# marksgraham/ddpm-ood

Measured on AMD Instinct MI355X. Metric: reconstructions/sec (whole node), FashionMNIST 32x32, higher is better.
Workload: dtype f32 (split-f16 MFMA products, fp32 accumulate)

## Files before the change

### ddpm_ood_amd/csrc/api.hip

```cpp
#include <stdarg.h>
#include <string.h>

#include <map>
#include <string>
#include <vector>

#include "common.h"

namespace ddpm {

static thread_local char g_err[512] = "";

void set_error(const char *fmt, ...) {
  va_list ap;
  va_start(ap, fmt);
  vsnprintf(g_err, sizeof(g_err), fmt, ap);
  va_end(ap);
}

static Switches g_sw;
static bool g_sw_loaded = false;
static unsigned g_sw_epoch = 0;
unsigned switch_epoch() { return g_sw_epoch; }
static int env_int(const char *name, int dflt) {
  const char *v = getenv(name);
  return v && *v ? atoi(v) : dflt;
}
static long env_long(const char *name, long dflt) {
  const char *v = getenv(name);
  return v && *v ? atol(v) : dflt;
}
static bool env_set(const char *name) { return getenv(name) != nullptr; }
static void load_switches() {
  const bool keep = g_sw.split_f16;
  Switches n;
  n.conv_wino44 = env_int("DDPM_CONV_WINO44", 1);
  n.wino44_f16x3 = env_int("DDPM_WINO44_F16X3", 1) != 0;
  n.wino44_split = env_int("DDPM_WINO44_SPLIT", 4);
  n.wino_split = env_int("DDPM_WINO_SPLIT", 8);
  n.w44h_xitem = env_int("DDPM_W44H_XITEM", 1);
  n.w44r_serp = env_int("DDPM_W44R_SERP", 0);
  n.wino44_xmap = env_int("DDPM_WINO44_XMAP", -1);
  n.up_wino44h = env_int("DDPM_UP_WINO44H", 1) != 0;
  n.down_s2h = env_int("DDPM_DOWN_S2H", 1);
  n.conv1x1_f16x3 = env_int("DDPM_CONV1X1_F16X3", 1) != 0;
  n.attn_f16x3 = env_int("DDPM_ATTN_F16X3", 1) != 0;
  n.wgrad_f16x3 = env_int("DDPM_WGRAD_F16X3", 1) != 0;
  n.attn_fa = env_int("DDPM_ATTN_FA", 1);
  n.conv_d3s = env_int("DDPM_CONV_D3S", 1);
  n.d1s_maxpx = env_int("DDPM_D1S_MAXPX", 16384);
  n.conv_splitk = env_int("DDPM_CONV_SPLITK", 1) != 0;
  n.conv_winograd = env_int("DDPM_CONV_WINOGRAD", 1) != 0;
  n.linear_skinny = env_int("DDPM_LINEAR_SKINNY", 1) != 0;
  n.conv1x1_dma = env_int("DDPM_CONV1X1_DMA", 1) != 0;
  n.gn_fused = env_int("DDPM_GN_FUSED", 1) != 0;
  n.attn_waves8 = env_int("DDPM_ATTN_WAVES", 8) != 4;
  n.convin_fast = env_int("DDPM_CONVIN_FAST", 1) != 0;
  n.convout_wave = env_int("DDPM_CONVOUT_WAVE", 1) != 0;
  n.convout_w16_maxwg = env_long("DDPM_CONVOUT_W16_MAXWG", -1);
  n.convin_blocks_per_cu = env_long("DDPM_CONVIN_BLOCKS_PER_CU", 8);
  n.gn_fwd_reg = env_int("DDPM_GN_FWD_REG", 1) != 0;
  n.gn_bwd_reg = env_int("DDPM_GN_BWD_REG", 1) != 0;
  n.gemm_v4 = env_int("DDPM_GEMM_V4", 1) != 0;
  n.gemm_f16x3 = env_int("DDPM_GEMM_F16X3", 1) != 0;
  n.wgrad_staged = env_int("DDPM_WGRAD_STAGED", 1) != 0;
  n.wgrad_waves8 = env_int("DDPM_WGRAD_WAVES", 8) != 4;
  n.gn_wave = env_int("DDPM_GN_WAVE", 1) != 0;
  n.conv1x1_dma_min_wg = env_long("DDPM_CONV1X1_DMA_MIN_WG", -1);
  n.conv1x1_xcd = env_int("DDPM_CONV1X1_XCD", 1) != 0;
  n.conv1x1_presplit = env_int("DDPM_CONV1X1_PRESPLIT", 1) != 0;
  n.conv_min_wg128 = env_long("DDPM_CONV_MIN_WG128", 512);
  n.conv_debug = env_set("DDPM_CONV_DEBUG");
  n.prof_shapes = env_set("DDPM_PROF_SHAPES");
  n.split_f16 = g_sw_loaded ? keep : true;
  g_sw = n;
  g_sw_loaded = true;
  g_sw_epoch += 1;
}
const Switches &sw() {
  if (!g_sw_loaded) load_switches();
  return g_sw;
}

static unsigned *g_status[64] = {};
unsigned *status_word() {
  int dev = 0;
  if (hipGetDevice(&dev) != hipSuccess || dev < 0 || dev >= 64) return nullptr;
  if (!g_status[dev]) {
    unsigned *p = nullptr;
    if (hipMalloc(&p, 256) != hipSuccess) return nullptr;
    if (hipMemset(p, 0, 256) != hipSuccess) {
      (void)hipFree(p);
      return nullptr;
    }
    g_status[dev] = p;
  }
  return g_status[dev];
}

struct ProfRec {
  hipEvent_t a, b;
  std::string kernel;
  double flops, bytes;
};
bool g_prof_on = false;
static std::vector<ProfRec> g_recs;

void prof_begin(hipStream_t s, const char *kernel, double flops, double bytes) {
  ProfRec r{nullptr, nullptr, std::string(kernel), flops, bytes};
  if (hipEventCreate(&r.a) != hipSuccess || hipEventCreate(&r.b) != hipSuccess) return;
  (void)hipEventRecord(r.a, s);
  g_recs.push_back(r);
}

void prof_end(hipStream_t s) {
  if (!g_recs.empty()) (void)hipEventRecord(g_recs.back().b, s);
}

}

using namespace ddpm;

extern "C" int ddpm_prof_enable(int on) {
  g_prof_on = on != 0;
  return 0;
}

extern "C" int ddpm_prof_report(char *buf, size_t cap) {
  struct Agg { long n = 0; double ms = 0, flops = 0, bytes = 0; };
  std::map<std::string, Agg> agg;
  for (auto &r : g_recs) {
    float ms = 0.f;
    if (hipEventSynchronize(r.b) == hipSuccess && hipEventElapsedTime(&ms, r.a, r.b) == hipSuccess) {
      Agg &a = agg[r.kernel];
      a.n += 1; a.ms += ms; a.flops += r.flops; a.bytes += r.bytes;
    }
    (void)hipEventDestroy(r.a);
    (void)hipEventDestroy(r.b);
  }
  g_recs.clear();
  std::string out = "{";
  bool first = true;
  for (auto &kv : agg) {
    char line[768];
    snprintf(line, sizeof(line), "%s\"%s\": {\"launches\": %ld, \"ms\": %.6f, \"flops\": %.6e, \"bytes\": %.6e}",
             first ? "" : ", ", kv.first.c_str(), kv.second.n, kv.second.ms, kv.second.flops, kv.second.bytes);
    out += line;
    first = false;
  }
  out += "}";
  if (!buf || out.size() + 1 > cap) {
    set_error("prof_report: buffer too small (%zu needed)", out.size() + 1);
    return DDPM_EINVAL;
  }
  memcpy(buf, out.c_str(), out.size() + 1);
  return (int)out.size();
}

extern "C" int ddpm_reload_env(void) {
  load_switches();
  return 0;
}

extern "C" int ddpm_set_split_f16(int on) {
  (void)sw();
  const int was = g_sw.split_f16 ? 1 : 0;
  if ((on != 0) != g_sw.split_f16) g_sw_epoch += 1;
  g_sw.split_f16 = on != 0;
  return was;
}

extern "C" int ddpm_get_split_f16(void) { return sw().split_f16 ? 1 : 0; }

extern "C" int ddpm_split_f16_active(void) {
  const Switches &w = sw();
  const bool any = w.wino44_f16x3 || w.conv1x1_f16x3 || w.attn_f16x3 || w.down_s2h != 0 || w.conv_d3s != 0 || w.up_wino44h;
  return w.split_f16 && any ? 1 : 0;
}

extern "C" int ddpm_status_read(unsigned *word, int clear, ddpm_stream_t stream) {
  DDPM_CHECK_ARG(word != nullptr, "status_read: NULL pointer");
  unsigned *st = status_word();
  DDPM_CHECK_ARG(st != nullptr, "status_read: no status word on this device");
  hipError_t e = hipMemcpyAsync(word, st, sizeof(unsigned), hipMemcpyDeviceToHost, as_stream(stream));
  if (e == hipSuccess && clear) e = hipMemsetAsync(st, 0, sizeof(unsigned), as_stream(stream));
  if (e == hipSuccess) e = hipStreamSynchronize(as_stream(stream));
  if (e != hipSuccess) {
    set_error("status_read: %s", hipGetErrorString(e));
    return (int)e;
  }
  return 0;
}

extern "C" int ddpm_abi_version(void) { return DDPM_ABI_VERSION; }
extern "C" const char *ddpm_last_error(void) { return g_err; }

extern "C" int ddpm_conv_f32(const ddpm_conv_desc *d, ddpm_stream_t stream) {
  DDPM_CHECK_ARG(d != nullptr, "conv: descriptor is NULL");
  return conv_dispatch(*d, as_stream(stream));
}

extern "C" size_t ddpm_conv_scratch_floats(const ddpm_conv_desc *d) {
  if (!d) return 0;
  return conv_scratch_floats(*d);
}

extern "C" size_t ddpm_conv_s2h_weight_halves(int Cout, int Cin) { return conv_s2h_weight_halves(Cout, Cin); }

extern "C" int ddpm_pack_conv_s2h_weight(const float *w_raw, uint16_t *dst, int Cout, int Cin, ddpm_stream_t stream) {
  return launch_pack_conv_s2h_weight(w_raw, dst, Cout, Cin, as_stream(stream));
}

extern "C" size_t ddpm_conv_d3h_weight_halves(int Cout, int Cin) { return conv_d3h_weight_halves(Cout, Cin); }

extern "C" size_t ddpm_conv_d1s_weight_halves(int Cout, int Cin) { return conv_d1s_weight_halves(Cout, Cin); }

extern "C" int ddpm_pack_conv_d1s_weight(const float *w_raw, uint16_t *dst, int Cout, int Cin, int cout_offset, int Cout_total,
                                         ddpm_stream_t stream) {
  return launch_pack_conv_d1s_weight(w_raw, dst, Cout, Cin, cout_offset, Cout_total, as_stream(stream));
}

extern "C" int ddpm_pack_conv_d3h_weight(const float *w_raw, uint16_t *dst, int Cout, int Cin, ddpm_stream_t stream) {
  return launch_pack_conv_d3h_weight(w_raw, dst, Cout, Cin, as_stream(stream));
}

extern "C" size_t ddpm_conv1x1_h_weight_halves(int Cout, int Cin) { return conv1x1_h_weight_halves(Cout, Cin); }

extern "C" int ddpm_pack_conv1x1_h_weight(const float *w_raw, uint16_t *dst, int Cout, int Cin, ddpm_stream_t stream) {
  return launch_pack_conv1x1_h_weight(w_raw, dst, Cout, Cin, 0, Cout, as_stream(stream));
}

extern "C" int ddpm_conv_stats_parts(const ddpm_conv_desc *d) {
  if (!d) return 0;
  return conv_stats_parts(*d);
}

extern "C" size_t ddpm_packed_conv_weight_floats(int Cout, int Cin, int ksize) {
  return packed_conv_weight_floats(Cout, Cin, ksize);
}

extern "C" int ddpm_pack_conv_weight_f32(const float *w_raw, float *w_packed, int Cout, int Cin, int ksize,
                                         int cout_offset, int Cout_total, ddpm_stream_t stream) {
  DDPM_CHECK_ARG(w_raw && w_packed, "pack: NULL pointer");
  return launch_pack_conv_weight(w_raw, w_packed, Cout, Cin, ksize, cout_offset, Cout_total, as_stream(stream));
}

extern "C" int ddpm_pack_conv_weight_taps_f32(const float *w_raw, float *w_packed, int Cout, int Cin, int ksize,
                                              int src_taps, int tap_off, ddpm_stream_t stream) {
  DDPM_CHECK_ARG(w_raw && w_packed && src_taps >= ksize * ksize && tap_off >= 0 && tap_off + ksize * ksize <= src_taps,
                 "pack_taps: bad argument");
  return launch_pack_conv_weight(w_raw, w_packed, Cout, Cin, ksize, 0, Cout, as_stream(stream), src_taps, tap_off);
}

extern "C" int ddpm_pack_conv3d_weight_f32(const float *w_raw, float *w_packed, int Cout, int Cin, int ksize,
                                           ddpm_stream_t stream) {
  DDPM_CHECK_ARG(w_raw && w_packed && (ksize == 3 || ksize == 4), "pack_conv3d: NULL pointer or ksize not 3 / 4");
  const size_t slab = (size_t)Cout * Cin * ksize * ksize;
  for (int kd = 0; kd < ksize; ++kd) {
    const int rc = launch_pack_conv_weight(w_raw, w_packed + kd * slab, Cout, Cin, ksize, 0, Cout, as_stream(stream),
                                           ksize * ksize * ksize, ksize * ksize * kd);
    if (rc) return rc;
  }
  return 0;
}

extern "C" size_t ddpm_packed_convtr_weight_floats(int Cout, int Cin, int dims) {
  return packed_convT_weight_floats(Cout, Cin, dims);
}

extern "C" int ddpm_pack_convtr_weight_f32(const float *w_raw, float *w_packed, int Cin, int Cout, int dims,
                                          ddpm_stream_t stream) {
  DDPM_CHECK_ARG(w_raw && w_packed, "pack_convT: NULL pointer");
  return launch_pack_convT_weight(w_raw, w_packed, Cin, Cout, dims, as_stream(stream));
}

extern "C" int ddpm_conv3d_k4s2_cin1_f32(const float *in, const float *w, const float *bias, float *out, int B,
                                         int Cout, int D, int H, int W, int relu, ddpm_stream_t stream) {
  return launch_conv3d_k4s2_cin1(in, w, bias, out, B, Cout, D, H, W, relu, as_stream(stream));
}

extern "C" int ddpm_convtr3d_k4s2_cout1_f32(const float *in, const float *w, const float *bias, float *out, int B,
                                           int Cin, int D, int H, int W, ddpm_stream_t stream) {
  return launch_convT3d_k4s2_cout1(in, w, bias, out, B, Cin, D, H, W, as_stream(stream));
}

extern "C" size_t ddpm_wino_weight_floats(int Cout, int Cin) { return wino_weight_floats(Cout, Cin); }

extern "C" int ddpm_pack_wino_weight_f32(const float *w_raw, float *w_wino, int Cout, int Cin, ddpm_stream_t stream) {
  DDPM_CHECK_ARG(w_raw && w_wino, "wino pack: NULL pointer");
  return launch_pack_wino_weight(w_raw, w_wino, Cout, Cin, as_stream(stream));
}

extern "C" size_t ddpm_wino44_weight_floats(int Cout, int Cin) { return wino44_weight_floats(Cout, Cin); }

extern "C" int ddpm_pack_wino44_weight_f32(const float *w_raw, float *w_wino44, int Cout, int Cin, ddpm_stream_t stream) {
  DDPM_CHECK_ARG(w_raw && w_wino44, "wino44 pack: NULL pointer");
  return launch_pack_wino44_weight(w_raw, w_wino44, Cout, Cin, as_stream(stream));
}

extern "C" int ddpm_convnd_generic_f32(const float *in, const float *w, const float *bias, const float *residual, float *out,
                                       int B, int Cin, int Cout, int Di, int Hi, int Wi, int dims, int ksize, int stride,
                                       int pad, int transposed, int relu, ddpm_stream_t stream) {
  return launch_convnd_generic(in, w, bias, residual, out, B, Cin, Cout, Di, Hi, Wi, dims, ksize, stride, pad, transposed, relu,
                               as_stream(stream));
}

extern "C" size_t ddpm_wino44h_weight_halves(int Cout, int Cin) { return wino44h_weight_halves(Cout, Cin); }

extern "C" int ddpm_pack_wino44h_weight(const float *w_raw, uint16_t *w_wino44h, int Cout, int Cin, ddpm_stream_t stream) {
  DDPM_CHECK_ARG(w_raw && w_wino44h, "wino44h pack: NULL pointer");
  return launch_pack_wino44h_weight(w_raw, w_wino44h, Cout, Cin, as_stream(stream));
}

extern "C" int ddpm_pack_wino44h_weight3d(const float *w_raw, uint16_t *w_wino44h, int Cout, int Cin, ddpm_stream_t stream) {
  DDPM_CHECK_ARG(w_raw && w_wino44h, "wino44h 3d pack: NULL pointer");
  return launch_pack_wino44h_weight(w_raw, w_wino44h, Cout, Cin, as_stream(stream), 3);
}

extern "C" int ddpm_pack_wino44_weight3d_f32(const float *w_raw, float *w_wino44, int Cout, int Cin, ddpm_stream_t stream) {
  DDPM_CHECK_ARG(w_raw && w_wino44, "wino44 3d pack: NULL pointer");
  return launch_pack_wino44_weight(w_raw, w_wino44, Cout, Cin, as_stream(stream), 3);
}

extern "C" int ddpm_pack_wino3d_weight_f32(const float *w_raw, float *w_wino, int Cout, int Cin, ddpm_stream_t stream) {
  DDPM_CHECK_ARG(w_raw && w_wino, "wino3d pack: NULL pointer");
  return launch_pack_wino_weight(w_raw, w_wino, Cout, Cin, as_stream(stream), 3);
}

extern "C" size_t ddpm_folded_upsample_weight_floats(int Cout, int Cin) {
  return folded_upsample_weight_floats(Cout, Cin);
}

extern "C" int ddpm_fold_upsample_weight_f32(const float *w_raw, float *w_folded, int Cout, int Cin,
                                             ddpm_stream_t stream) {
  DDPM_CHECK_ARG(w_raw && w_folded, "fold: NULL pointer");
  return launch_fold_upsample_weight(w_raw, w_folded, Cout, Cin, as_stream(stream));
}

extern "C" int ddpm_gn_finalize_f32(const float *st1, int parts1, int C1, const float *st2, int parts2, int C2,
                                    const float *gamma, const float *beta, float *scale, float *shift, int B, int HW,
                                    int groups, float eps, ddpm_stream_t stream) {
  return launch_gn_finalize(st1, parts1, C1, st2, parts2, C2, gamma, beta, scale, shift, B, HW, groups, eps,
                            as_stream(stream));
}

extern "C" int ddpm_channel_stats_f32(const float *in, float *stats, int B, int C, int HW, ddpm_stream_t stream) {
  return launch_channel_stats(in, stats, B, C, HW, as_stream(stream));
}

extern "C" int ddpm_gn_scale_shift_f32(const float *in1, const float *in2, int C1, int C2, const float *gamma,
                                       const float *beta, float *scale, float *shift, int B, int HW, int groups,
                                       float eps, ddpm_stream_t stream) {
  return launch_gn_scale_shift(in1, in2, C1, C2, gamma, beta, scale, shift, B, HW, groups, eps, as_stream(stream));
}

extern "C" int ddpm_attention_f32(const float *qkv, const float *residual, float *out, int B, int C, int N,
                                  int num_heads, float scale, ddpm_stream_t stream) {
  return launch_attention(qkv, residual, out, B, C, N, num_heads, scale, as_stream(stream));
}

extern "C" size_t ddpm_attention_scratch_floats(int B, int C, int N, int num_heads) {
  return attention_fa_scratch_floats(B, C, N, num_heads);
}

extern "C" int ddpm_attention_ws_f32(const float *qkv, const float *residual, float *out, int B, int C, int N, int num_heads,
                                     float scale, float *scratch, size_t scratch_floats, ddpm_stream_t stream) {
  return launch_attention(qkv, residual, out, B, C, N, num_heads, scale, as_stream(stream), scratch, scratch_floats);
}

extern "C" int ddpm_attention_train_fwd_f32(const float *q, const float *k, const float *v, float *o, float *lse, int B, int C, int N,
                                            int num_heads, float scale, ddpm_stream_t stream) {
  return launch_attention_train_fwd(q, k, v, o, lse, B, C, N, num_heads, scale, as_stream(stream));
}

extern "C" int ddpm_attention_train_bwd_f32(const float *q, const float *k, const float *v, const float *o, const float *dout,
                                            const float *lse, float *delta, float *dq, float *dk, float *dv, int B, int C, int N,
                                            int num_heads, float scale, ddpm_stream_t stream) {
  return launch_attention_train_bwd(q, k, v, o, dout, lse, delta, dq, dk, dv, B, C, N, num_heads, scale, as_stream(stream));
}
```

### ddpm_ood_amd/csrc/common.h

```cpp
#pragma once
#include <hip/hip_runtime.h>
#include <stdint.h>
#include <stdio.h>
#include <string>

#include "../../include/ddpm_ood_hip.h"

namespace ddpm {

void set_error(const char *fmt, ...);

inline hipStream_t as_stream(ddpm_stream_t s) { return reinterpret_cast<hipStream_t>(s); }

#define DDPM_CHECK_ARG(cond, ...)                \
  do {                                           \
    if (!(cond)) {                               \
      ::ddpm::set_error(__VA_ARGS__);            \
      return DDPM_EINVAL;                        \
    }                                            \
  } while (0)

#define DDPM_CHECK_LAUNCH()                                                    \
  do {                                                                         \
    hipError_t e_ = hipGetLastError();                                         \
    if (e_ != hipSuccess) {                                                    \
      ::ddpm::set_error("%s:%d: %s", __FILE__, __LINE__, hipGetErrorString(e_)); \
      return (int)e_;                                                          \
    }                                                                          \
  } while (0)

constexpr int kWave = 64;

struct Switches {
  int conv_wino44 = 1;
  bool wino44_f16x3 = true;
  int wino44_split = 4;
  int wino_split = 8;
  int wino44_xmap = -1;
  int w44r_serp = 0;
  int w44h_xitem = 1;
  bool up_wino44h = true;
  int down_s2h = 1;
  bool conv1x1_f16x3 = true;
  bool attn_f16x3 = true;
  int d1s_maxpx = 16384;
  int conv_d3s = 1;
  int attn_fa = 1;
  bool conv_splitk = true;
  bool conv_winograd = true;
  bool linear_skinny = true;
  bool conv1x1_dma = true;
  bool gn_fused = true;
  bool attn_waves8 = true;
  bool convin_fast = true;
  bool convout_wave = true;
  long convout_w16_maxwg = -1;
  long convin_blocks_per_cu = 8;
  bool wgrad_f16x3 = true;
  bool gn_fwd_reg = true;
  bool gn_bwd_reg = true;
  bool gemm_v4 = true;
  bool gemm_f16x3 = true;
  bool wgrad_staged = true;
  bool wgrad_waves8 = true;
  bool gn_wave = true;
  long conv1x1_dma_min_wg = -1;
  bool conv1x1_xcd = true;
  bool conv1x1_presplit = true;
  long conv_min_wg128 = 512;
  bool conv_debug = false;
  bool prof_shapes = false;
  bool split_f16 = true;
};
const Switches &sw();
unsigned switch_epoch();
inline bool split_f16_on(bool family) { return family && sw().split_f16; }

unsigned *status_word();
__device__ __forceinline__ bool non_finite(float v) { return !(__builtin_fabsf(v) <= 3.402823466e+38f); }

__device__ __forceinline__ void philox_round(uint32_t (&c)[4], uint32_t (&k)[2]) {
  const uint64_t p0 = (uint64_t)0xD2511F53u * c[0], p1 = (uint64_t)0xCD9E8D57u * c[2];
  const uint32_t n0 = (uint32_t)(p1 >> 32) ^ c[1] ^ k[0], n1 = (uint32_t)p1, n2 = (uint32_t)(p0 >> 32) ^ c[3] ^ k[1], n3 = (uint32_t)p0;
  c[0] = n0; c[1] = n1; c[2] = n2; c[3] = n3;
  k[0] += 0x9E3779B9u;
  k[1] += 0xBB67AE85u;
}
__device__ __forceinline__ void philox_normal4(int64_t q, uint64_t stream, uint64_t seed, float (&z)[4]) {
  uint32_t c[4] = {(uint32_t)q, (uint32_t)((uint64_t)q >> 32), (uint32_t)stream, (uint32_t)(stream >> 32)};
  uint32_t k[2] = {(uint32_t)seed, (uint32_t)(seed >> 32)};
#pragma unroll
  for (int r = 0; r < 10; ++r) philox_round(c, k);
#pragma unroll
  for (int h = 0; h < 2; ++h) {
    const float u1 = ((float)c[2 * h] + 1.0f) * 2.3283064365386963e-10f;
    const float u2 = (float)c[2 * h + 1] * 2.3283064365386963e-10f;
    const float rad = sqrtf(-2.0f * logf(u1 < 1e-30f ? 1e-30f : u1));
    float sn, cs;
    sincosf(6.283185307179586f * u2, &sn, &cs);
    z[2 * h] = rad * cs;
    z[2 * h + 1] = rad * sn;
  }
}

extern bool g_prof_on;
void prof_begin(hipStream_t s, const char *kernel, double flops, double bytes);
void prof_end(hipStream_t s);
struct ProfScope {
  hipStream_t s;
  bool on;
  ProfScope(hipStream_t st, const char *kernel, double flops, double bytes) : s(st), on(g_prof_on) {
    if (on) prof_begin(s, kernel, flops, bytes);
  }
  ~ProfScope() {
    if (on) prof_end(s);
  }
};

__device__ __forceinline__ float relu_f(float v) { return v < 0.f ? 0.f : v; }
__device__ __forceinline__ float max_keep_nan(float m, float v) { return (v > m || v != v) ? v : m; }

__device__ __forceinline__ float silu_f(float v) { return v / (1.0f + expf(-v)); }
__device__ __forceinline__ float silu_fast(float v) {
  return v * __builtin_amdgcn_rcpf(1.0f + __builtin_amdgcn_exp2f(-1.44269504088896341f * v));
}

__device__ __forceinline__ float wave_sum(float v) {
#pragma unroll
  for (int o = 32; o > 0; o >>= 1) v += __shfl_xor(v, o, 64);
  return v;
}
template <int CTRL>
__device__ __forceinline__ float dpp_mov0(float v) {
  return __builtin_bit_cast(float, __builtin_amdgcn_update_dpp(0, __builtin_bit_cast(int, v), CTRL, 0xf, 0xf, true));
}
template <int CTRL>
__device__ __forceinline__ void chan_merge_dpp(float &mean, float &m2, float &halfn) {
  const float mo = dpp_mov0<CTRL>(mean), qo = dpp_mov0<CTRL>(m2);
  const float dl = mo - mean;
  m2 = (m2 + qo) + dl * dl * halfn;
  mean = 0.5f * (mean + mo);
  halfn += halfn;
}
__device__ __forceinline__ float wave_sum_dpp_last_lane(float v) {
  v += dpp_mov0<0x111>(v);
  v += dpp_mov0<0x112>(v);
  v += dpp_mov0<0x114>(v);
  v += dpp_mov0<0x118>(v);
  v += dpp_mov0<0x142>(v);
  v += dpp_mov0<0x143>(v);
  return v;
}
__device__ __forceinline__ void group_moments_last_lane(float &mean, float &m2, float cnt, int lanes) {
  float halfn = 0.5f * cnt;
  chan_merge_dpp<0x111>(mean, m2, halfn);
  chan_merge_dpp<0x112>(mean, m2, halfn);
  if (lanes > 4) {
    chan_merge_dpp<0x114>(mean, m2, halfn);
    chan_merge_dpp<0x118>(mean, m2, halfn);
  }
  if (lanes > 16) chan_merge_dpp<0x142>(mean, m2, halfn);
  if (lanes > 32) chan_merge_dpp<0x143>(mean, m2, halfn);
}
__device__ __forceinline__ float wave_max(float v) {
#pragma unroll
  for (int o = 32; o > 0; o >>= 1) v = fmaxf(v, __shfl_xor(v, o, 64));
  return v;
}

typedef _Float16 f16x8 __attribute__((ext_vector_type(8)));

constexpr float kF16LoScale = 32.f;

__device__ __forceinline__ void split_f16x8(const float (&v)[8], f16x8 &hi, f16x8 &lo, f16x8 &hs) {
#pragma unroll
  for (int t = 0; t < 8; ++t) {
    const _Float16 h = (_Float16)v[t];
    hi[t] = h;
    lo[t] = (_Float16)((v[t] - (float)h) * kF16LoScale);
  }
  hs = hi * (_Float16)(1.f / kF16LoScale);
}

#define DDPM_MFMA_F16X3(acc, ah, al, as, bh, bl, bs)                              \
  do {                                                                            \
    (acc) = __builtin_amdgcn_mfma_f32_32x32x16_f16((as), (bl), (acc), 0, 0, 0);   \
    (acc) = __builtin_amdgcn_mfma_f32_32x32x16_f16((al), (bs), (acc), 0, 0, 0);   \
    (acc) = __builtin_amdgcn_mfma_f32_32x32x16_f16((ah), (bh), (acc), 0, 0, 0);   \
  } while (0)

__device__ __forceinline__ float block_sum_256(float v, float *red) {
  v = wave_sum(v);
  const int lane = threadIdx.x & 63, wave = threadIdx.x >> 6;
  __syncthreads();
  if (lane == 0) red[wave] = v;
  __syncthreads();
  return (red[0] + red[1]) + (red[2] + red[3]);
}

int device_cus();
int conv_dispatch(const ddpm_conv_desc &d, hipStream_t s);
size_t conv_scratch_floats(const ddpm_conv_desc &d);
int conv_stats_parts(const ddpm_conv_desc &d);
bool linear_skinny_supported(const ddpm_conv_desc &d);
int launch_linear_skinny(const ddpm_conv_desc &d, hipStream_t s);
bool conv_d3s_supported(const ddpm_conv_desc &d);
int launch_conv_d3s(const ddpm_conv_desc &d, hipStream_t s);
size_t conv_d3s_scratch_floats(const ddpm_conv_desc &d);
int conv_d3s_stats_parts(const ddpm_conv_desc &d);
bool conv_d3s2_supported(const ddpm_conv_desc &d);
int launch_conv_d3s2(const ddpm_conv_desc &d, hipStream_t s);
size_t conv_d3s2_scratch_floats(const ddpm_conv_desc &d);
bool conv_d1s_supported(const ddpm_conv_desc &d);
int launch_conv_d1s(const ddpm_conv_desc &d, hipStream_t s);
size_t conv_d1s_scratch_floats(const ddpm_conv_desc &d);
size_t conv_d3h_weight_halves(int Cout, int Cin);
int launch_pack_conv_d3h_weight(const float *w_raw, uint16_t *dst, int Cout, int Cin, hipStream_t s);
size_t conv_d1s_weight_halves(int Cout, int Cin);
int launch_pack_conv_d1s_weight(const float *w_raw, uint16_t *dst, int Cout, int Cin, int cout_offset, int Cout_total, hipStream_t s);
bool conv_wino44h_supported(const ddpm_conv_desc &d);
int launch_conv_wino44h(const ddpm_conv_desc &d, hipStream_t s);
size_t conv_wino44h_scratch_floats(const ddpm_conv_desc &d);
int conv_wino44h_stats_parts(const ddpm_conv_desc &d);
size_t wino44h_weight_halves(int Cout, int Cin);
int launch_pack_wino44h_weight(const float *w_raw, uint16_t *w_wino44h, int Cout, int Cin, hipStream_t s, int nkd = 1);
bool conv_wino44_supported(const ddpm_conv_desc &d);
int launch_conv_wino44(const ddpm_conv_desc &d, hipStream_t s);
size_t conv_wino44_scratch_floats(const ddpm_conv_desc &d);
size_t wino44_weight_floats(int Cout, int Cin);
bool conv_wino_supported(const ddpm_conv_desc &d);
int launch_conv_wino(const ddpm_conv_desc &d, hipStream_t s);
size_t conv_wino_scratch_floats(const ddpm_conv_desc &d);
int conv_wino_stats_parts(const ddpm_conv_desc &d);
size_t wino_weight_floats(int Cout, int Cin);
int launch_wino_split_reduce(const ddpm_conv_desc &d, int S, long long pstride, int HW, hipStream_t s);
int wino_split_reduce_stats_parts(int HW);
bool conv_s2h_supported(const ddpm_conv_desc &d);
int launch_conv_s2h(const ddpm_conv_desc &d, hipStream_t s);
int conv_s2h_stats_parts(const ddpm_conv_desc &d);
size_t conv_s2h_weight_halves(int Cout, int Cin);
int launch_pack_conv_s2h_weight(const float *w_raw, uint16_t *dst, int Cout, int Cin, hipStream_t s);
bool conv1x1_dma_supported(const ddpm_conv_desc &d);
int launch_conv1x1_dma(const ddpm_conv_desc &d, hipStream_t s);
size_t conv1x1_h_weight_halves(int Cout, int Cin);
int launch_pack_conv1x1_h_weight(const float *w_raw, uint16_t *dst, int Cout, int Cin, int cout_offset, int Cout_total,
                                 hipStream_t s);
bool conv_mfma_supported(const ddpm_conv_desc &d);
int launch_conv_mfma(const ddpm_conv_desc &d, hipStream_t s);
size_t conv_mfma_scratch_floats(const ddpm_conv_desc &d);
size_t packed_conv_weight_floats(int Cout, int Cin, int ksize);
size_t folded_upsample_weight_floats(int Cout, int Cin);
bool conv_direct_supported(const ddpm_conv_desc &d);
int launch_conv_direct(const ddpm_conv_desc &d, hipStream_t s);
int conv_direct_stats_parts(const ddpm_conv_desc &d);
int launch_pack_wino44_weight(const float *w_raw, float *w_wino44, int Cout, int Cin, hipStream_t s, int nkd = 1);
int launch_pack_wino_weight(const float *w_raw, float *w_wino, int Cout, int Cin, hipStream_t s, int nkd = 1);
int launch_fold_upsample_weight(const float *w_raw, float *w_folded, int Cout, int Cin, hipStream_t s);
int launch_pack_conv_weight(const float *w_raw, float *w_packed, int Cout, int Cin, int ksize, int cout_offset,
                            int Cout_total, hipStream_t s, int src_taps = 0, int tap_off = 0);
size_t packed_convT_weight_floats(int Cout, int Cin, int dims);
int launch_pack_convT_weight(const float *w_raw, float *w_packed, int Cin, int Cout, int dims, hipStream_t s);
int launch_conv3d_k4s2_cin1(const float *in, const float *w, const float *bias, float *out, int B, int Cout, int D,
                            int H, int W, int relu, hipStream_t s);
int launch_convT3d_k4s2_cout1(const float *in, const float *w, const float *bias, float *out, int B, int Cin, int D,
                              int H, int W, hipStream_t s);
int launch_convnd_generic(const float *in, const float *w, const float *bias, const float *residual, float *out, int B, int Cin,
                          int Cout, int Di, int Hi, int Wi, int dims, int k, int stride, int pad, int transposed, int relu,
                          hipStream_t s);
int launch_gn_scale_shift(const float *in1, const float *in2, int C1, int C2, const float *gamma, const float *beta,
                          float *scale, float *shift, int B, int HW, int groups, float eps, hipStream_t s);
int launch_gn_finalize(const float *st1, int parts1, int C1, const float *st2, int parts2, int C2, const float *gamma,
                       const float *beta, float *scale, float *shift, int B, int HW, int groups, float eps, hipStream_t s);
int launch_channel_stats(const float *in, float *stats, int B, int C, int HW, hipStream_t s);
int launch_attention(const float *qkv, const float *residual, float *out, int B, int C, int N, int heads, float scale,
                     hipStream_t s, float *scratch = nullptr, size_t scratch_floats = 0, float *stats_out = nullptr);
bool attention_emits_stats(int B, int C, int N, int heads, const float *scratch, size_t scratch_floats);
size_t attention_fa_scratch_floats(int B, int C, int N, int heads);
bool attention_fa_supported(int B, int C, int N, int heads, const float *scratch, size_t scratch_floats);
int launch_attention_fa(const float *qkv, const float *residual, float *out, int B, int C, int N, int heads, float scale,
                        float *scratch, hipStream_t s);
int launch_attention_train_fwd(const float *q, const float *k, const float *v, float *o, float *lse, int B, int C, int N, int heads,
                               float scale, hipStream_t s);
int launch_attention_train_bwd(const float *q, const float *k, const float *v, const float *o, const float *dout, const float *lse,
                               float *delta, float *dq, float *dk, float *dv, int B, int C, int N, int heads, float scale,
                               hipStream_t s);
int launch_timestep_embedding(const int64_t *t, const float *freqs, float *out, int B, int dim, hipStream_t s);
int launch_copy_f32(const float *src, float *dst, int64_t n, hipStream_t s);

constexpr int kConvCc = 4;
constexpr int kConvNT = 128;
constexpr int kConvMT = 128;

}
```

### ddpm_ood_amd/csrc/conv1x1_dma.hip

```cpp
#include "common.h"

namespace ddpm {

typedef float f32x16 __attribute__((ext_vector_type(16)));
constexpr float kF16WScale = 64.f;

constexpr int kDC = 16;
constexpr int kDM = 128;
constexpr int kDP = 256;
constexpr int kDBuf = kDC * (kDM + kDP);
constexpr int kDAff = 4 * 64;

static bool conv1x1_f16x3_enabled() {
  return split_f16_on(sw().conv1x1_f16x3);
}

bool conv1x1_dma_supported(const ddpm_conv_desc &d) {
  const int Cin = d.C1 + d.C2;
  const long HW = (long)d.Ho * d.Wo;
  if (!sw().conv1x1_dma || d.force_direct || !d.w_packed) return false;
  if (d.ksize != 1 || d.mode != DDPM_CONV_NORMAL || d.act != DDPM_ACT_NONE) return false;
  if (d.gscale && (!conv1x1_f16x3_enabled() || !d.gshift || HW % 64)) return false;
  if (d.Di > 1 || d.Do > 1) return false;
  if (Cin % kDC || (d.C2 > 0 && d.C1 % kDC) || d.Cout % kDM) return false;
  if (HW % 4 || !((HW % kDP == 0) || (kDP % HW == 0))) return false;
  const long tiles = ((long)d.B * HW + kDP - 1) / kDP;
  const long min_wg_env = sw().conv1x1_dma_min_wg;
  const long min_wg = min_wg_env >= 0 ? min_wg_env
                      : conv1x1_f16x3_enabled() ? 64
                                                : 384;
  return tiles * (d.Cout / kDM) >= min_wg;
}

template <bool F16X3, bool AFFINE, bool PRE = false>
__global__ __launch_bounds__(256, 2) void conv1x1_dma_kernel(const ddpm_conv_desc a) {
  static_assert(!PRE || F16X3, "pre-split weights are the split-f16 form's");
  constexpr int NI = PRE ? 4 : 2, NJ = PRE ? 2 : 4;
  extern __shared__ __attribute__((aligned(16))) float smem[];
  constexpr int kBuf = kDBuf + (AFFINE ? kDAff : 0);
  const int tid = threadIdx.x;
  const int lane = tid & 63, wave = __builtin_amdgcn_readfirstlane(tid >> 6);
  const int l31 = lane & 31, lhi = lane >> 5;
  const int wco = PRE ? 0 : (wave & 1) * 64, wpx = PRE ? wave * 64 : (wave >> 1) * 128;
  const int HW = a.Ho * a.Wo, Cin = a.C1 + a.C2, nchunks = Cin / kDC;
  int nt;
  long t0;
  {
    const unsigned CT = a.Cout / kDM, PT = (unsigned)(((long)a.B * a.Ho * a.Wo + kDP - 1) / kDP);
    unsigned ptile;
    if (gridDim.y == 1) {
      const unsigned xcd = blockIdx.x & 7, m = blockIdx.x >> 3;
      ptile = (m / CT) * 8 + xcd;
      nt = m % CT;
    } else {
      ptile = blockIdx.x;
      nt = blockIdx.y;
    }
    if (ptile >= PT) return;
    t0 = (long)ptile * kDP;
  }
  const long npix = (long)a.B * HW;

  const float *wsrc = (PRE ? reinterpret_cast<const float *>(a.w_wino44h) : a.w_packed) + (size_t)nt * nchunks * kDC * kDM +
                      wave * 512 + lane * 4;
  size_t boff1, boff2;
  {
    long t = t0 + lane * 4;
    if (t >= npix) t = npix - 4;
    const long n = t / HW, p = t - n * HW;
    boff1 = ((size_t)n * a.C1) * HW + p;
    boff2 = ((size_t)n * a.C2) * HW + p;
  }
  const float *gsrc = nullptr;
  if constexpr (AFFINE) {
    long n = (t0 + 64 * wave) / HW;
    if (n >= a.B) n = a.B - 1;
    gsrc = ((lane & 16) ? a.gshift : a.gscale) + (size_t)n * Cin + (lane & 15);
  }
  auto dma_chunk = [&](int q, int buf) {
    float *dstA = smem + buf * kBuf;
    float *dstB = dstA + kDC * kDM;
#pragma unroll
    for (int j = 0; j < 2; ++j)
      __builtin_amdgcn_global_load_lds(wsrc + (size_t)q * kDC * kDM + j * 256, dstA + wave * 512 + j * 256, 16, 0, 0);
#pragma unroll
    for (int j = 0; j < 4; ++j) {
      const int c = 4 * wave + j, cg = q * kDC + c;
      const bool first = cg < a.C1;
      const float *src = first ? a.in1 + boff1 + (size_t)cg * HW : a.in2 + boff2 + (size_t)(cg - a.C1) * HW;
      __builtin_amdgcn_global_load_lds(src, dstB + c * kDP, 16, 0, 0);
    }
    if constexpr (AFFINE) __builtin_amdgcn_global_load_lds(gsrc + q * kDC, dstA + kDBuf + wave * 64, 4, 0, 0);
  };

  f32x16 acc[NI][NJ];
#pragma unroll
  for (int i = 0; i < NI; ++i)
#pragma unroll
    for (int j = 0; j < NJ; ++j)
#pragma unroll
      for (int r = 0; r < 16; ++r) acc[i][j][r] = 0.f;

  dma_chunk(0, 0);
  if (nchunks > 1) dma_chunk(1, 1);
  for (int q = 0; q < nchunks; ++q) {
    if (q + 1 < nchunks) {
      if constexpr (AFFINE)
        asm volatile("s_waitcnt vmcnt(7)\n\ts_barrier" ::: "memory");
      else
        asm volatile("s_waitcnt vmcnt(6)\n\ts_barrier" ::: "memory");
    } else
      asm volatile("s_waitcnt vmcnt(0)\n\ts_barrier" ::: "memory");
    if (q + 2 < nchunks) dma_chunk(q + 2, (q + 2) % 3);
    if constexpr (F16X3) {
      const float *A = smem + (q % 3) * kBuf + 8 * lhi * kDM + wco + l31;
      const float *Bm = smem + (q % 3) * kBuf + kDC * kDM + 8 * lhi * kDP + wpx + l31;
      const float *G = smem + (q % 3) * kBuf + kDBuf + (wpx >> 6) * 64 + 8 * lhi;
      f16x8 ah[NI], al[NI], as[NI];
      if constexpr (PRE) {
        const f16x8 *Ah = reinterpret_cast<const f16x8 *>(smem + (q % 3) * kBuf) + lhi * kDM + l31, *Al = Ah + 2 * kDM;
#pragma unroll
        for (int i = 0; i < NI; ++i) {
          ah[i] = Ah[32 * i];
          al[i] = Al[32 * i];
          as[i] = ah[i] * (_Float16)(1.f / kF16LoScale);
        }
      } else {
#pragma unroll
        for (int i = 0; i < NI; ++i) {
          float v[8];
#pragma unroll
          for (int t = 0; t < 8; ++t) v[t] = A[t * kDM + 32 * i] * kF16WScale;
          split_f16x8(v, ah[i], al[i], as[i]);
        }
      }
      float bq[2][8];
#pragma unroll
      for (int t = 0; t < 8; ++t) bq[0][t] = Bm[t * kDP];
      float sc[8], sh[8];
#pragma unroll
      for (int j = 0; j < NJ; ++j) {
        if (j + 1 < NJ) {
#pragma unroll
          for (int t = 0; t < 8; ++t) bq[(j + 1) & 1][t] = Bm[t * kDP + 32 * (j + 1)];
        }
        if constexpr (AFFINE) {
          if ((j & 1) == 0) {
#pragma unroll
            for (int t = 0; t < 8; ++t) {
              sc[t] = G[(j >> 1) * 64 + t];
              sh[t] = G[(j >> 1) * 64 + 16 + t];
            }
          }
#pragma unroll
          for (int t = 0; t < 8; ++t) bq[j & 1][t] = bq[j & 1][t] * sc[t] + sh[t];
        }
        f16x8 bh, bl, bs;
        split_f16x8(bq[j & 1], bh, bl, bs);
#pragma unroll
        for (int i = 0; i < NI; ++i) acc[i][j] = __builtin_amdgcn_mfma_f32_32x32x16_f16(as[i], bl, acc[i][j], 0, 0, 0);
#pragma unroll
        for (int i = 0; i < NI; ++i) acc[i][j] = __builtin_amdgcn_mfma_f32_32x32x16_f16(al[i], bs, acc[i][j], 0, 0, 0);
#pragma unroll
        for (int i = 0; i < NI; ++i) acc[i][j] = __builtin_amdgcn_mfma_f32_32x32x16_f16(ah[i], bh, acc[i][j], 0, 0, 0);
      }
    } else {
      const float *A = smem + (q % 3) * kBuf + lhi * kDM + wco + l31;
      const float *Bm = A - (lhi * kDM + wco + l31) + kDC * kDM + lhi * kDP + wpx + l31;
      float av[2][2], bv[2][4];
      auto fetch = [&](int ks, int slot) {
#pragma unroll
        for (int i = 0; i < 2; ++i) av[slot][i] = A[2 * ks * kDM + 32 * i];
#pragma unroll
        for (int j = 0; j < 4; ++j) bv[slot][j] = Bm[2 * ks * kDP + 32 * j];
      };
      fetch(0, 0);
#pragma unroll
      for (int ks = 0; ks < kDC / 2; ++ks) {
        if (ks + 1 < kDC / 2) fetch(ks + 1, (ks + 1) & 1);
        __builtin_amdgcn_sched_barrier(0);
#pragma unroll
        for (int i = 0; i < 2; ++i)
#pragma unroll
          for (int j = 0; j < 4; ++j)
            acc[i][j] = __builtin_amdgcn_mfma_f32_32x32x2f32(av[ks & 1][i], bv[ks & 1][j], acc[i][j], 0, 0, 0);
        __builtin_amdgcn_sched_barrier(0);
      }
    }
  }

  const int co_base = nt * kDM + wco + 4 * lhi;
#pragma unroll
  for (int j = 0; j < NJ; ++j) {
    const long t = t0 + wpx + 32 * j + l31;
    if (t < npix) {
      const long n = t / HW, p = t - n * HW;
      const size_t obase = ((size_t)n * a.Cout + co_base) * HW + p;
#pragma unroll
      for (int i = 0; i < NI; ++i) {
        float add[16], rv[16];
#pragma unroll
        for (int r = 0; r < 16; ++r) {
          const int dco = 32 * i + (r & 3) + 8 * (r >> 2);
          add[r] = (a.bias ? a.bias[co_base + dco] : 0.f) +
                   (a.chan_add ? a.chan_add[(size_t)n * a.chan_add_stride + co_base + dco] : 0.f);
          rv[r] = a.residual ? a.residual[obase + (size_t)dco * HW] : 0.f;
        }
#pragma unroll
        for (int r = 0; r < 16; ++r) {
          const int dco = 32 * i + (r & 3) + 8 * (r >> 2);
          float v = acc[i][j][r];
          if constexpr (F16X3) v *= 1.f / kF16WScale;
          if (a.bias || a.chan_add) v += add[r];
          if (a.residual) v += rv[r];
          if (a.out_act == DDPM_ACT_RELU) v = relu_f(v);
          a.out[obase + (size_t)dco * HW] = v;
        }
      }
    }
  }
}

__global__ void conv1x1_h_pack_kernel(const float *__restrict__ src, _Float16 *__restrict__ dst, int Cout, int Cin, int cout_offset,
                                      int Cout_total) {
  const int64_t total = (int64_t)Cout * Cin;
  const int nchunks = Cin / kDC;
  for (int64_t i = blockIdx.x * (int64_t)blockDim.x + threadIdx.x; i < total; i += (int64_t)gridDim.x * blockDim.x) {
    const int ci = (int)(i % Cin), co = (int)(i / Cin) + cout_offset;
    const float v = src[i] * kF16WScale;
    const _Float16 h = (_Float16)v;
    const _Float16 l = (_Float16)((v - (float)h) * kF16LoScale);
    const int tile = co / kDM, c128 = co % kDM, chunk = ci / kDC, kk = ci % kDC;
    const size_t unit = (((size_t)tile * nchunks + chunk) * 2 * 2 + (kk >> 3)) * kDM + c128;
    dst[unit * 8 + (kk & 7)] = h;
    dst[(unit + 2 * kDM) * 8 + (kk & 7)] = l;
  }
  (void)Cout_total;
}

size_t conv1x1_h_weight_halves(int Cout, int Cin) {
  return (Cout % kDM == 0 && Cin % kDC == 0) ? (size_t)Cout * Cin * 2 : 0;
}

int launch_pack_conv1x1_h_weight(const float *w_raw, uint16_t *dst, int Cout, int Cin, int cout_offset, int Cout_total,
                                 hipStream_t s) {
  DDPM_CHECK_ARG(w_raw && dst && conv1x1_h_weight_halves(Cout_total, Cin) != 0 && cout_offset >= 0 && cout_offset + Cout <= Cout_total,
                 "conv1x1 pre-split pack: Cout_total %% 128 or Cin %% 16 != 0, or rows out of range");
  const int64_t total = (int64_t)Cout * Cin;
  hipLaunchKernelGGL(conv1x1_h_pack_kernel, dim3((unsigned)((total + 255) / 256)), dim3(256), 0, s, w_raw,
                     reinterpret_cast<_Float16 *>(dst), Cout, Cin, cout_offset, Cout_total);
  DDPM_CHECK_LAUNCH();
  return 0;
}

int launch_conv1x1_dma(const ddpm_conv_desc &d, hipStream_t s) {
  if (!conv1x1_dma_supported(d)) {
    set_error("conv1x1_dma: unsupported shape");
    return DDPM_EINVAL;
  }
  const bool f16x3 = conv1x1_f16x3_enabled(), aff = d.gscale != nullptr;
  const size_t lds = (size_t)3 * (kDBuf + (aff ? kDAff : 0)) * sizeof(float);
  static bool attr_done = false;
  if (!attr_done) {
    for (const void *f : {reinterpret_cast<const void *>(&conv1x1_dma_kernel<false, false>),
                          reinterpret_cast<const void *>(&conv1x1_dma_kernel<true, false>),
                          reinterpret_cast<const void *>(&conv1x1_dma_kernel<true, true>),
                          reinterpret_cast<const void *>(&conv1x1_dma_kernel<true, false, true>),
                          reinterpret_cast<const void *>(&conv1x1_dma_kernel<true, true, true>)})
      (void)hipFuncSetAttribute(f, hipFuncAttributeMaxDynamicSharedMemorySize, 160 * 1024);
    attr_done = true;
  }
  const long HW = (long)d.Ho * d.Wo, npix = (long)d.B * HW;
  const int Cin = d.C1 + d.C2;
  ProfScope prof(s, aff ? "conv1x1_dma_gn" : "conv1x1_dma", 2.0 * npix * d.Cout * Cin,
                 4.0 * ((double)npix * Cin + (double)npix * d.Cout * (d.residual ? 2 : 1) + (double)d.Cout * Cin));
  const unsigned PT = (unsigned)((npix + kDP - 1) / kDP), CT = d.Cout / kDM;
  const dim3 grid = sw().conv1x1_xcd ? dim3(8 * ((PT + 7) / 8) * CT) : dim3(PT, CT);
  const bool pre = f16x3 && sw().conv1x1_presplit && d.w_wino44h != nullptr;
  if (pre && aff)
    hipLaunchKernelGGL((conv1x1_dma_kernel<true, true, true>), grid, dim3(256), lds, s, d);
  else if (pre)
    hipLaunchKernelGGL((conv1x1_dma_kernel<true, false, true>), grid, dim3(256), lds, s, d);
  else if (aff)
    hipLaunchKernelGGL((conv1x1_dma_kernel<true, true>), grid, dim3(256), lds, s, d);
  else if (f16x3)
    hipLaunchKernelGGL((conv1x1_dma_kernel<true, false>), grid, dim3(256), lds, s, d);
  else
    hipLaunchKernelGGL((conv1x1_dma_kernel<false, false>), grid, dim3(256), lds, s, d);
  DDPM_CHECK_LAUNCH();
  return 0;
}

}
```

Before: 1103.

## Add 256-cout by 128-pixel tile variant for pre-split 1x1 conv kernel

Adds a WIDE template variant of the 1x1 conv DMA kernel. Each workgroup covers 256 output channels by 128 pixels instead of 128 by 256, and each wave computes 8 M-tiles against a single 32-pixel column. The activation tile is split to f16 once per wave and reused across more weight tiles. The variant is used when Cout is a multiple of 256 and the weights are pre-split. The trade-off is more weight traffic per pixel, a different grid size and more accumulator registers per wave, which could affect occupancy.

Result: no change. 1107 (median of 6 runs) (+0.4%).

```diff
diff --git a/ddpm_ood_amd/csrc/api.hip b/ddpm_ood_amd/csrc/api.hip
--- a/ddpm_ood_amd/csrc/api.hip
+++ b/ddpm_ood_amd/csrc/api.hip
@@ -69,6 +69,7 @@
   n.conv1x1_dma_min_wg = env_long("DDPM_CONV1X1_DMA_MIN_WG", -1);
   n.conv1x1_xcd = env_int("DDPM_CONV1X1_XCD", 1) != 0;
   n.conv1x1_presplit = env_int("DDPM_CONV1X1_PRESPLIT", 1) != 0;
+  n.conv1x1_wide = env_int("DDPM_CONV1X1_WIDE", 1) != 0;
   n.conv_min_wg128 = env_long("DDPM_CONV_MIN_WG128", 512);
   n.conv_debug = env_set("DDPM_CONV_DEBUG");
   n.prof_shapes = env_set("DDPM_PROF_SHAPES");
diff --git a/ddpm_ood_amd/csrc/common.h b/ddpm_ood_amd/csrc/common.h
--- a/ddpm_ood_amd/csrc/common.h
+++ b/ddpm_ood_amd/csrc/common.h
@@ -67,6 +67,7 @@
   long conv1x1_dma_min_wg = -1;
   bool conv1x1_xcd = true;
   bool conv1x1_presplit = true;
+  bool conv1x1_wide = true;
   long conv_min_wg128 = 512;
   bool conv_debug = false;
   bool prof_shapes = false;
diff --git a/ddpm_ood_amd/csrc/conv1x1_dma.hip b/ddpm_ood_amd/csrc/conv1x1_dma.hip
--- a/ddpm_ood_amd/csrc/conv1x1_dma.hip
+++ b/ddpm_ood_amd/csrc/conv1x1_dma.hip
@@ -32,21 +32,24 @@
   return tiles * (d.Cout / kDM) >= min_wg;
 }
 
-template <bool F16X3, bool AFFINE, bool PRE = false>
+template <bool F16X3, bool AFFINE, bool PRE = false, bool WIDE = false>
 __global__ __launch_bounds__(256, 2) void conv1x1_dma_kernel(const ddpm_conv_desc a) {
   static_assert(!PRE || F16X3, "pre-split weights are the split-f16 form's");
-  constexpr int NI = PRE ? 4 : 2, NJ = PRE ? 2 : 4;
+  static_assert(!WIDE || PRE, "the 256-cout workgroup takes pre-split weights");
+  constexpr int kM = WIDE ? 2 * kDM : kDM, kP = WIDE ? kDP / 2 : kDP;
+  constexpr int NI = WIDE ? 8 : PRE ? 4 : 2, NJ = WIDE ? 1 : PRE ? 2 : 4;
   extern __shared__ __attribute__((aligned(16))) float smem[];
   constexpr int kBuf = kDBuf + (AFFINE ? kDAff : 0);
   const int tid = threadIdx.x;
   const int lane = tid & 63, wave = __builtin_amdgcn_readfirstlane(tid >> 6);
   const int l31 = lane & 31, lhi = lane >> 5;
-  const int wco = PRE ? 0 : (wave & 1) * 64, wpx = PRE ? wave * 64 : (wave >> 1) * 128;
+  const int wco = PRE ? 0 : (wave & 1) * 64;
+  const int wpx = WIDE ? wave * 32 : PRE ? wave * 64 : (wave >> 1) * 128;
   const int HW = a.Ho * a.Wo, Cin = a.C1 + a.C2, nchunks = Cin / kDC;
   int nt;
   long t0;
   {
-    const unsigned CT = a.Cout / kDM, PT = (unsigned)(((long)a.B * a.Ho * a.Wo + kDP - 1) / kDP);
+    const unsigned CT = a.Cout / kM, PT = (unsigned)(((long)a.B * a.Ho * a.Wo + kP - 1) / kP);
     unsigned ptile;
     if (gridDim.y == 1) {
       const unsigned xcd = blockIdx.x & 7, m = blockIdx.x >> 3;
@@ -57,15 +60,17 @@
       nt = blockIdx.y;
     }
     if (ptile >= PT) return;
-    t0 = (long)ptile * kDP;
+    t0 = (long)ptile * kP;
   }
   const long npix = (long)a.B * HW;
 
-  const float *wsrc = (PRE ? reinterpret_cast<const float *>(a.w_wino44h) : a.w_packed) + (size_t)nt * nchunks * kDC * kDM +
-                      wave * 512 + lane * 4;
+  const float *wsrc = (PRE ? reinterpret_cast<const float *>(a.w_wino44h) : a.w_packed) +
+                      (WIDE ? (size_t)(2 * nt + (wave >> 1)) * nchunks * kDC * kDM + (wave & 1) * 1024
+                            : (size_t)nt * nchunks * kDC * kDM + wave * 512) +
+                      lane * 4;
   size_t boff1, boff2;
   {
-    long t = t0 + lane * 4;
+    long t = t0 + (WIDE ? l31 : lane) * 4;
     if (t >= npix) t = npix - 4;
     const long n = t / HW, p = t - n * HW;
     boff1 = ((size_t)n * a.C1) * HW + p;
@@ -73,22 +78,34 @@
   }
   const float *gsrc = nullptr;
   if constexpr (AFFINE) {
-    long n = (t0 + 64 * wave) / HW;
+    long n = (t0 + 64 * (WIDE ? wave >> 1 : wave)) / HW;
     if (n >= a.B) n = a.B - 1;
     gsrc = ((lane & 16) ? a.gshift : a.gscale) + (size_t)n * Cin + (lane & 15);
   }
   auto dma_chunk = [&](int q, int buf) {
     float *dstA = smem + buf * kBuf;
-    float *dstB = dstA + kDC * kDM;
-#pragma unroll
-    for (int j = 0; j < 2; ++j)
-      __builtin_amdgcn_global_load_lds(wsrc + (size_t)q * kDC * kDM + j * 256, dstA + wave * 512 + j * 256, 16, 0, 0);
-#pragma unroll
-    for (int j = 0; j < 4; ++j) {
-      const int c = 4 * wave + j, cg = q * kDC + c;
-      const bool first = cg < a.C1;
+    float *dstB = dstA + kDC * kM;
+    if constexpr (WIDE) {
+#pragma unroll
+      for (int j = 0; j < 4; ++j)
+        __builtin_amdgcn_global_load_lds(wsrc + (size_t)q * kDC * kDM + j * 256, dstA + wave * 1024 + j * 256, 16, 0, 0);
+      const int cg = q * kDC + 4 * wave + lhi;
+      const bool first = q * kDC < a.C1;
       const float *src = first ? a.in1 + boff1 + (size_t)cg * HW : a.in2 + boff2 + (size_t)(cg - a.C1) * HW;
-      __builtin_amdgcn_global_load_lds(src, dstB + c * kDP, 16, 0, 0);
+#pragma unroll
+      for (int j = 0; j < 2; ++j)
+        __builtin_amdgcn_global_load_lds(src + (size_t)2 * j * HW, dstB + (4 * wave + 2 * j) * kP, 16, 0, 0);
+    } else {
+#pragma unroll
+      for (int j = 0; j < 2; ++j)
+        __builtin_amdgcn_global_load_lds(wsrc + (size_t)q * kDC * kDM + j * 256, dstA + wave * 512 + j * 256, 16, 0, 0);
+#pragma unroll
+      for (int j = 0; j < 4; ++j) {
+        const int c = 4 * wave + j, cg = q * kDC + c;
+        const bool first = cg < a.C1;
+        const float *src = first ? a.in1 + boff1 + (size_t)cg * HW : a.in2 + boff2 + (size_t)(cg - a.C1) * HW;
+        __builtin_amdgcn_global_load_lds(src, dstB + c * kDP, 16, 0, 0);
+      }
     }
     if constexpr (AFFINE) __builtin_amdgcn_global_load_lds(gsrc + q * kDC, dstA + kDBuf + wave * 64, 4, 0, 0);
   };
@@ -112,7 +129,36 @@
     } else
       asm volatile("s_waitcnt vmcnt(0)\n\ts_barrier" ::: "memory");
     if (q + 2 < nchunks) dma_chunk(q + 2, (q + 2) % 3);
-    if constexpr (F16X3) {
+    if constexpr (WIDE) {
+      const float *Bm = smem + (q % 3) * kBuf + kDC * kM + 8 * lhi * kP + wpx + l31;
+      float bq[8];
+#pragma unroll
+      for (int t = 0; t < 8; ++t) bq[t] = Bm[t * kP];
+      if constexpr (AFFINE) {
+        const float *G = smem + (q % 3) * kBuf + kDBuf + wave * 64 + 8 * lhi;
+#pragma unroll
+        for (int t = 0; t < 8; ++t) bq[t] = bq[t] * G[t] + G[16 + t];
+      }
+      f16x8 bh, bl, bs;
+      split_f16x8(bq, bh, bl, bs);
+      const f16x8 *Ah = reinterpret_cast<const f16x8 *>(smem + (q % 3) * kBuf) + lhi * kDM + l31, *Al = Ah + 2 * kDM;
+#pragma unroll
+      for (int g = 0; g < 2; ++g) {
+        f16x8 ah[4], al[4], as[4];
+#pragma unroll
+        for (int i = 0; i < 4; ++i) {
+          ah[i] = Ah[g * 4 * kDM + 32 * i];
+          al[i] = Al[g * 4 * kDM + 32 * i];
+          as[i] = ah[i] * (_Float16)(1.f / kF16LoScale);
+        }
+#pragma unroll
+        for (int i = 0; i < 4; ++i) acc[4 * g + i][0] = __builtin_amdgcn_mfma_f32_32x32x16_f16(as[i], bl, acc[4 * g + i][0], 0, 0, 0);
+#pragma unroll
+        for (int i = 0; i < 4; ++i) acc[4 * g + i][0] = __builtin_amdgcn_mfma_f32_32x32x16_f16(al[i], bs, acc[4 * g + i][0], 0, 0, 0);
+#pragma unroll
+        for (int i = 0; i < 4; ++i) acc[4 * g + i][0] = __builtin_amdgcn_mfma_f32_32x32x16_f16(ah[i], bh, acc[4 * g + i][0], 0, 0, 0);
+      }
+    } else if constexpr (F16X3) {
       const float *A = smem + (q % 3) * kBuf + 8 * lhi * kDM + wco + l31;
       const float *Bm = smem + (q % 3) * kBuf + kDC * kDM + 8 * lhi * kDP + wpx + l31;
       const float *G = smem + (q % 3) * kBuf + kDBuf + (wpx >> 6) * 64 + 8 * lhi;
@@ -189,7 +235,7 @@
     }
   }
 
-  const int co_base = nt * kDM + wco + 4 * lhi;
+  const int co_base = nt * kM + wco + 4 * lhi;
 #pragma unroll
   for (int j = 0; j < NJ; ++j) {
     const long t = t0 + wpx + 32 * j + l31;
@@ -266,7 +312,9 @@
                           reinterpret_cast<const void *>(&conv1x1_dma_kernel<true, false>),
                           reinterpret_cast<const void *>(&conv1x1_dma_kernel<true, true>),
                           reinterpret_cast<const void *>(&conv1x1_dma_kernel<true, false, true>),
-                          reinterpret_cast<const void *>(&conv1x1_dma_kernel<true, true, true>)})
+                          reinterpret_cast<const void *>(&conv1x1_dma_kernel<true, true, true>),
+                          reinterpret_cast<const void *>(&conv1x1_dma_kernel<true, false, true, true>),
+                          reinterpret_cast<const void *>(&conv1x1_dma_kernel<true, true, true, true>)})
       (void)hipFuncSetAttribute(f, hipFuncAttributeMaxDynamicSharedMemorySize, 160 * 1024);
     attr_done = true;
   }
@@ -274,10 +322,16 @@
   const int Cin = d.C1 + d.C2;
   ProfScope prof(s, aff ? "conv1x1_dma_gn" : "conv1x1_dma", 2.0 * npix * d.Cout * Cin,
                  4.0 * ((double)npix * Cin + (double)npix * d.Cout * (d.residual ? 2 : 1) + (double)d.Cout * Cin));
-  const unsigned PT = (unsigned)((npix + kDP - 1) / kDP), CT = d.Cout / kDM;
+  const bool pre = f16x3 && sw().conv1x1_presplit && d.w_wino44h != nullptr;
+  const bool wide = pre && sw().conv1x1_wide && d.Cout % (2 * kDM) == 0 && (HW % (kDP / 2) == 0 || (kDP / 2) % HW == 0);
+  const long P = wide ? kDP / 2 : kDP;
+  const unsigned PT = (unsigned)((npix + P - 1) / P), CT = d.Cout / (wide ? 2 * kDM : kDM);
   const dim3 grid = sw().conv1x1_xcd ? dim3(8 * ((PT + 7) / 8) * CT) : dim3(PT, CT);
-  const bool pre = f16x3 && sw().conv1x1_presplit && d.w_wino44h != nullptr;
-  if (pre && aff)
+  if (wide && aff)
+    hipLaunchKernelGGL((conv1x1_dma_kernel<true, true, true, true>), grid, dim3(256), lds, s, d);
+  else if (wide)
+    hipLaunchKernelGGL((conv1x1_dma_kernel<true, false, true, true>), grid, dim3(256), lds, s, d);
+  else if (pre && aff)
     hipLaunchKernelGGL((conv1x1_dma_kernel<true, true, true>), grid, dim3(256), lds, s, d);
   else if (pre)
     hipLaunchKernelGGL((conv1x1_dma_kernel<true, false, true>), grid, dim3(256), lds, s, d);
```
